# PaddleCV-SIG/MedicalSeg

Hardware: AMD Instinct MI355X
Metric: 3D-voxels/sec fwd+bwd, VNet 128^3 fp32 (higher is better)
Workload: dtype f32

## Files before the change

### include/msegk.h

```cpp
#ifndef MSEGK_H
#define MSEGK_H

#include <stddef.h>
#include <stdint.h>

#ifdef __cplusplus
extern "C" {
#endif

typedef struct msk_ctx msk_ctx;

typedef struct {
  void* p;
  int32_t n, d, h, w, c;
  int32_t ld;
} msk_tensor;

typedef struct {
  int32_t kd, kh, kw;
  int32_t sd, sh, sw;
  int32_t pd, ph, pw;
} msk_conv_desc;

int msk_version(void);
// ... 79 lines not shown
                                 const float* alpha, const float* mean, const float* invstd, msk_tensor dout, float* sums,
                                 float* maxes , int clear_maxes, float* dgamma, float* dbeta, float* dalpha);
int msk_add_act_join_bwd_pg(msk_ctx* ctx, msk_tensor y, const float* scale, const float* shift, const float* alpha_inner,
                            msk_tensor res, const float* alpha_outer, const float* mean, const float* invstd, msk_tensor dout,
                            msk_tensor da, msk_tensor dres, int dres_accumulate, float* dalpha_outer, float* unit_sums,
                            float* maxes , int clear_maxes, float* unit_dgamma, float* unit_dbeta, float* unit_dalpha);
size_t msk_conv3d_bwd_bnact_bytes(msk_ctx* ctx, msk_conv_desc cd, msk_tensor x, msk_tensor y);
int msk_conv3d_bwd_bnact(msk_ctx* ctx, msk_conv_desc cd, msk_tensor x, const float* w, msk_tensor y, const float* scale,
                         const float* shift, const float* alpha , const float* mean, const float* invstd,
                         const float* gamma, msk_tensor dout, const float* sums_total, double M_total,
                         msk_tensor dy_scratch, msk_tensor dx, int dx_accumulate, float* dw, int dw_accumulate,
                         const void* xform , void* ybuf ,
                         const float* maxes );
int msk_conv3d_bwd_bnact_split(msk_ctx* ctx, msk_conv_desc cd, msk_tensor x, const float* w, msk_tensor y, const float* scale,
                               const float* shift, const float* alpha , const float* mean, const float* invstd,
                               const float* gamma, msk_tensor dout, const float* sums_total, double M_total,
                               msk_tensor dy_scratch, msk_tensor dx, int dx_accumulate, float* dw, int dw_accumulate,
                               const void* xform , void* ybuf , const float* maxes ,
                               msk_tensor dx_lo, msk_tensor dx_hi, int* split_done);
int msk_conv3d_bwd_bnact_acc(msk_ctx* ctx, msk_conv_desc cd, msk_tensor x, const float* w, msk_tensor y, const float* scale,
                             const float* shift, const float* alpha, const float* mean, const float* invstd, const float* gamma,
                             msk_tensor dout, const float* sums_total, double M_total, msk_tensor dy_scratch, msk_tensor dx,
                             int dx_accumulate, float* dw, int dw_accumulate, const void* xform, void* ybuf, const float* maxes,
                             msk_tensor dx_old, msk_tensor dx_lo, msk_tensor dx_hi, int* split_done);
int msk_conv3d_bwd_bnact_join(msk_ctx* ctx, msk_conv_desc cd, msk_tensor x, const float* w, msk_tensor y, const float* scale,
                              const float* shift, const float* alpha , const float* mean, const float* invstd,
                              const float* gamma, msk_tensor dout, const float* sums_total, double M_total, msk_tensor dy,
                              float* dy_amax , float* dw, int dw_accumulate, const void* xform ,
                              const float* x_amax , msk_tensor jy, const float* jscale, const float* jshift,
                              const float* jalpha_inner, msk_tensor jres, const float* jalpha_outer, const float* jmean,
                              const float* jinvstd, msk_tensor da, int da_accumulate, msk_tensor dres ,
                              int dres_accumulate, float* dalpha_outer, float* unit_sums, float* maxes, int clear_maxes,
                              float* unit_dgamma , float* unit_dbeta , float* unit_dalpha );
int msk_convT3d_bwd_bnact(msk_ctx* ctx, msk_conv_desc cd, msk_tensor x, const float* w, msk_tensor y, const float* scale,
                          const float* shift, const float* alpha , const float* mean, const float* invstd,
                          msk_tensor dout, const float* sums_total, double M_total, msk_tensor dy_scratch, msk_tensor dx,
                          int dx_accumulate, float* dw, int dw_accumulate);
int msk_conv3d_bwd_inact(msk_ctx* ctx, msk_conv_desc cd, msk_tensor x, const float* w, msk_tensor y, const float* scale,
                         const float* shift, const float* alpha , const float* mean, const float* invstd, int coef_stride,
                         msk_tensor dout, const float* sums, int sums_stride, double M_sample, msk_tensor dx, int dx_accumulate,
                         float* dw, int dw_accumulate, const void* xform, void* ybuf, const float* maxes );
int msk_conv3d_bwd_bnact_c1(msk_ctx* ctx, msk_conv_desc cd, msk_tensor x, msk_tensor y, const float* scale, const float* shift,
                            const float* alpha , const float* mean, const float* invstd, msk_tensor res,
                            msk_tensor dout, const float* sums_total, double M_total, float* dw, int dw_accumulate);
int msk_conv3d_dgrad(msk_ctx* ctx, msk_conv_desc cd, msk_tensor dy, const float* w,
                     msk_tensor dx, int accumulate);
int msk_conv3d_wgrad(msk_ctx* ctx, msk_conv_desc cd, msk_tensor x, msk_tensor dy,
                     float* dw, float* db , int accumulate);
int msk_convT3d_fwd(msk_ctx* ctx, msk_conv_desc cd, msk_tensor x, const float* w,
                    const float* bias , msk_tensor y);
int msk_convT3d_fwd_ex(msk_ctx* ctx, msk_conv_desc cd, msk_tensor x, const float* w, const float* bias, msk_tensor y,
                       float* stats_local, const msk_bn_fin* fin );
int msk_convT3d_dgrad(msk_ctx* ctx, msk_conv_desc cd, msk_tensor dy, const float* w,
                      msk_tensor dx, int accumulate);
int msk_convT3d_wgrad(msk_ctx* ctx, msk_conv_desc cd, msk_tensor x, msk_tensor dy,
                      float* dw, float* db , int accumulate);

int msk_bn_stats(msk_ctx* ctx, msk_tensor x, float* stats_local);
int msk_bn_finalize(msk_ctx* ctx, const float* gathered, int world, double count_per_rank,
                    int C, const float* gamma, const float* beta, float eps, float momentum,
                    float* running_mean, float* running_var, float* save_mean,
                    float* save_invstd, float* scale, float* shift);
int msk_bn_eval_coeffs(msk_ctx* ctx, int C, const float* gamma, const float* beta,
                       const float* running_mean, const float* running_var, float eps,
                       float* save_mean, float* save_invstd, float* scale, float* shift);
int msk_affine_act_fwd(msk_ctx* ctx, msk_tensor x, const float* scale, const float* shift,
// ... 230 lines not shown
```

### medicalseg_amd/_lib.py

```python
from __future__ import annotations

import ctypes as C
import os

_HERE = os.path.dirname(os.path.abspath(__file__))
LIB_PATH = os.environ.get("MSEGK_LIB") or os.path.join(_HERE, "lib", "libmsegk.so")


class MskError(RuntimeError):
    pass


class MskTensor(C.Structure):
    _fields_ = [("p", C.c_void_p), ("n", C.c_int32), ("d", C.c_int32), ("h", C.c_int32),
                ("w", C.c_int32), ("c", C.c_int32), ("ld", C.c_int32)]


class MskConvDesc(C.Structure):
    _fields_ = [("kd", C.c_int32), ("kh", C.c_int32), ("kw", C.c_int32),
                ("sd", C.c_int32), ("sh", C.c_int32), ("sw", C.c_int32),
                ("pd", C.c_int32), ("ph", C.c_int32), ("pw", C.c_int32)]


class MskBnFin(C.Structure):
# ... 36 lines not shown
    "msk_mark_elapsed": (_i, [_vp, _i, _i, C.POINTER(_f)]),
    "msk_prof_enable": (_i, [_vp, _i]),
    "msk_prof_reset": (_i, [_vp]),
    "msk_prof_report": (_i, [_vp, C.c_char_p, _i, C.POINTER(_i)]),
    "msk_set_option": (_i, [_vp, C.c_char_p, _i]),
    "msk_get_option": (_i, [_vp, C.c_char_p, C.POINTER(_i)]),
    "msk_ncdhw_to_ndhwc": (_i, [_vp, _vp, _T]),
    "msk_ndhwc_to_ncdhw": (_i, [_vp, _T, _vp]),
    "msk_conv3d_fwd": (_i, [_vp, _CD, _T, _vp, _vp, _T]),
    "msk_conv_fold_bn": (_i, [_vp, _vp, _vp, _vp, _vp, _i, C.c_long, _vp, _vp]),
    "msk_conv3d_fwd_act": (_i, [_vp, _CD, _T, _vp, _vp, _vp, _T]),
    "msk_conv3d_xform_bytes": (_sz, [_vp, _CD, _T, _i]),
    "msk_conv3d_fwd_ex": (_i, [_vp, _CD, _T, _vp, _vp, _T, _vp, _vp]),
    "msk_conv3d_wgrad_ex": (_i, [_vp, _CD, _T, _T, _vp, _vp, _i, _vp]),
    "msk_amax_new": (_vp, [_vp, _i]),
    "msk_conv3d_fwd_ex3": (_i, [_vp, _CD, _T, _vp, _vp, _T, _vp, _vp, _vp, _vp]),
    "msk_conv3d_fwd_in": (_i, [_vp, _CD, _T, _vp, _vp, _T, _vp, _vp, _vp, _vp, _i]),
    "msk_bn_stats_fin": (_i, [_vp, _T, _vp, _vp]),
    "msk_affine_act_bwd_reduce_pg": (_i, [_vp, _T, _vp, _vp, _T, _vp, _vp, _vp, _T, _vp, _vp, _i, _vp, _vp, _vp]),
    "msk_add_act_join_bwd_pg": (_i, [_vp, _T, _vp, _vp, _vp, _T, _vp, _vp, _vp, _T, _T, _T, _i, _vp, _vp, _vp, _i, _vp, _vp, _vp]),
    "msk_conv3d_fwd_ex2": (_i, [_vp, _CD, _T, _vp, _vp, _T, _vp, _vp, _vp]),
    "msk_affine_act_fwd_amax": (_i, [_vp, _T, _vp, _vp, _T, _vp, _T, _vp]),
    "msk_affine_act_fwd_amax2": (_i, [_vp, _T, _vp, _vp, _T, _vp, _T, _vp, _T]),
    "msk_affine_act_join_fwd_amax": (_i, [_vp, _T, _vp, _vp, _vp, _T, _vp, _T, _vp]),
    "msk_copy_scale_amax": (_i, [_vp, _T, _vp, _T, _i, _vp]),
    "msk_conv3d_bwd_bnact_bytes": (_sz, [_vp, _CD, _T, _T]),
    "msk_conv3d_bwd_bnact": (_i, [_vp, _CD, _T, _vp, _T, _vp, _vp, _vp, _vp, _vp, _vp, _T, _vp, _d, _T, _T, _i, _vp, _i, _vp, _vp, _vp]),
    "msk_convT3d_bwd_bnact": (_i, [_vp, _CD, _T, _vp, _T, _vp, _vp, _vp, _vp, _vp, _T, _vp, _d, _T, _T, _i, _vp, _i]),
    "msk_conv3d_bwd_bnact_split": (_i, [_vp, _CD, _T, _vp, _T, _vp, _vp, _vp, _vp, _vp, _vp, _T, _vp, _d, _T, _T, _i, _vp, _i, _vp, _vp, _vp, _T, _T, C.POINTER(_i)]),
    "msk_conv3d_bwd_bnact_acc": (_i, [_vp, _CD, _T, _vp, _T, _vp, _vp, _vp, _vp, _vp, _vp, _T, _vp, _d, _T, _T, _i, _vp, _i, _vp, _vp, _vp, _T, _T, _T, C.POINTER(_i)]),
    "msk_conv3d_bwd_inact": (_i, [_vp, _CD, _T, _vp, _T, _vp, _vp, _vp, _vp, _vp, _i, _T, _vp, _i, _d, _T, _i, _vp, _i, _vp, _vp, _vp]),
    "msk_conv3d_bwd_bnact_join": (_i, [_vp, _CD, _T, _vp, _T, _vp, _vp, _vp, _vp, _vp, _vp, _T, _vp, _d, _T, _vp, _vp, _i, _vp, _vp,
                                       _T, _vp, _vp, _vp, _T, _vp, _vp, _vp, _T, _i, _T, _i, _vp, _vp, _vp, _i, _vp, _vp, _vp]),
    "msk_conv3d_bwd_bnact_c1": (_i, [_vp, _CD, _T, _T, _vp, _vp, _vp, _vp, _vp, _T, _T, _vp, _d, _vp, _i]),
    "msk_conv3d_dgrad": (_i, [_vp, _CD, _T, _vp, _T, _i]),
    "msk_conv3d_dgrad_ex": (_i, [_vp, _CD, _T, _vp, _T, _i, _vp]),
    "msk_conv3d_wgrad_ex2": (_i, [_vp, _CD, _T, _T, _vp, _vp, _i, _vp, _vp]),
    "msk_conv3d_wgrad_ex3": (_i, [_vp, _CD, _T, _T, _vp, _vp, _i, _vp, _vp, _vp]),
    "msk_conv3d_wgrad": (_i, [_vp, _CD, _T, _T, _vp, _vp, _i]),
    "msk_convT3d_fwd": (_i, [_vp, _CD, _T, _vp, _vp, _T]),
    "msk_convT3d_fwd_ex": (_i, [_vp, _CD, _T, _vp, _vp, _T, _vp, _vp]),
    "msk_convT3d_dgrad": (_i, [_vp, _CD, _T, _vp, _T, _i]),
    "msk_convT3d_wgrad": (_i, [_vp, _CD, _T, _T, _vp, _vp, _i]),
    "msk_bn_stats": (_i, [_vp, _T, _vp]),
    "msk_bn_finalize": (_i, [_vp, _vp, _i, _d, _i, _vp, _vp, _f, _f, _vp, _vp, _vp, _vp, _vp, _vp]),
    "msk_bn_eval_coeffs": (_i, [_vp, _i, _vp, _vp, _vp, _vp, _f, _vp, _vp, _vp, _vp]),
    "msk_affine_act_fwd": (_i, [_vp, _T, _vp, _vp, _T, _vp, _T]),
    "msk_affine_act_bwd_reduce": (_i, [_vp, _T, _vp, _vp, _T, _vp, _vp, _vp, _T, _vp]),
    "msk_affine_act_bwd_reduce_ex": (_i, [_vp, _T, _vp, _vp, _T, _vp, _vp, _vp, _T, _vp, _vp]),
    "msk_affine_act_bwd_apply": (_i, [_vp, _T, _vp, _vp, _T, _vp, _vp, _vp, _vp, _T, _vp, _d, _i, _T, _T, _i]),
    "msk_affine_act_bwd_apply_amax": (_i, [_vp, _T, _vp, _vp, _T, _vp, _vp, _vp, _vp, _T, _vp, _d, _i, _T, _T, _i, _vp]),
    "msk_affine_act_param_grads": (_i, [_vp, _i, _vp, _vp, _vp, _vp, _i]),
    "msk_add_act_bwd": (_i, [_vp, _T, _T, _vp, _T, _T, _T, _i, _vp]),
    "msk_affine_act_join_fwd": (_i, [_vp, _T, _vp, _vp, _vp, _T, _vp, _T]),
    "msk_add_act_join_bwd": (_i, [_vp, _T, _vp, _vp, _vp, _T, _vp, _T, _T, _T, _i, _vp]),
    "msk_add_act_join_bwd_ex": (_i, [_vp, _T, _vp, _vp, _vp, _T, _vp, _vp, _vp, _T, _T, _T, _i, _vp, _vp, _vp]),
    "msk_bn_bias_grad": (_i, [_vp, _i, _vp, _vp, _vp, _i]),
    "msk_copy_scale": (_i, [_vp, _T, _vp, _T, _i]),
    "msk_dropout_mask": (_i, [_vp, _u64, _u64, _u32, _i, _f, _vp]),
    "msk_channel_sum": (_i, [_vp, _T, _vp, _i]),
    "msk_argmax_c": (_i, [_vp, _T, _vp]),
    "msk_softmax_c": (_i, [_vp, _T, _T]),
    "msk_flip_axes": (_i, [_vp, _T, _T, _i]),
    "msk_tta_accumulate": (_i, [_vp, _T, _i, _T, _i]),
    "msk_tta_finish": (_i, [_vp, _T, _i, _T, _vp]),
    "msk_sw_gather": (_i, [_vp, _T, _T, _vp, _f]),
# ... 120 lines not shown
```

### medicalseg_amd/csrc/msk_common.h

```cpp
#pragma once
#include <hip/hip_runtime.h>
#include <hip/hip_ext.h>

#include <cstdint>
#include <cstdio>
#include <cstring>
#include <map>
#include <set>
#include <string>
#include <utility>
#include <vector>

#include "msegk.h"

struct msk_prof_entry {
  double total_ms = 0.0;
  long calls = 0;
};

struct msk_pending_event {
  hipEvent_t a, b;
  const char* tag;
};

// ... 87 lines not shown
  struct { float* param = nullptr; const float* grad = nullptr; float* velocity = nullptr; size_t count = 0;
           float lr = 0, momentum = 0, weight_decay = 0, grad_scale = 0; } late_piece;
  int late_split = 1;
  bool wgrad_async = false;
  bool side_dirty = false;
  hipEvent_t fork_event = nullptr;
  int fork_attach = 1;
  bool fork_recorded = false;
  void* stage[2] = {nullptr, nullptr};
  size_t stage_bytes[2] = {0, 0};
  hipEvent_t stage_ev[2] = {nullptr, nullptr};
  int stage_next = 0;
  void* comm = nullptr;
  void* comm_grad = nullptr;
  hipStream_t comm_stream = nullptr;
  hipEvent_t ev_comm_main = nullptr, ev_comm_side = nullptr, ev_comm_done = nullptr, ev_comm_back = nullptr;
  int c1_h2 = 1;
  int dst_split = 1;
  int wgrad_reduce_rows = 1;
  int ks_stats = 1;
  int ks_lds = 1;
  int ks_nr_max = 4;
  int wgrad_lds_pad = 0;
  int kst_pair = 1;
  int tile_staging = 7;
  int wgrad_renorm = 1;
  int dy_bound_shift = 0;
  int dp_mode = 0;
  bool comm_pending = false;
  bool host_transport = false;
  std::vector<int> host_fds;
  int rank = 0, world = 1;
  int tk_join = 1;
  int topk_agg_hist = 0;
  int affine_map = 1;
  int num_cu = 256;
};

extern thread_local std::string g_msk_global_err;

int msk_fail(msk_ctx* ctx, const char* file, int line, const char* what, const char* detail);
void* msk_workspace(msk_ctx* ctx, size_t bytes);
void* msk_workspace2(msk_ctx* ctx, size_t bytes);
void* msk_workspace3(msk_ctx* ctx, size_t bytes);
hipEvent_t msk_prof_event(msk_ctx* ctx);
void msk_prof_begin(msk_ctx* ctx, const char* tag);
void msk_prof_end(msk_ctx* ctx);
const char* msk_intern_tag(msk_ctx* ctx, const std::string& s);
int msk_join_side_impl(msk_ctx* ctx);
void msk_set_dense12(int v);
void msk_set_reduce_vpl(int v);
void msk_set_reduce_vpl_site(int v);
void msk_set_ew_caps(int ew, int red);
int msk_get_ew_option(const char* key, int* value);
void msk_weights_changed_impl(msk_ctx* ctx, const void* p, size_t bytes);
void msk_weights_freed_impl(msk_ctx* ctx, const void* p, size_t bytes);
int msk_prepack_impl(msk_ctx* ctx);
int msk_prepack_range_impl(msk_ctx* ctx, const void* p, size_t bytes);
int msk_dp_wait_impl(msk_ctx* ctx);
int msk_edt_field(msk_ctx* ctx, const int32_t* vol, int d, int h, int w, int cls, int surface_only, int complement,
                  const double* spacing, double* dist2);
int msk_join_sums_merge(msk_ctx* ctx, const float* partial, int nb, int C, float* unit_sums, float* u_dbeta, float* u_dgamma,
                        float* u_dalpha, float* dalpha);

struct msk_side_scope {
  msk_ctx* ctx;
// ... 91 lines not shown
```

### medicalseg_amd/csrc/msk_ctx.hip

```cpp
#include <cstdlib>

#include "msk_common.h"

thread_local std::string g_msk_global_err;

int msk_fail(msk_ctx* ctx, const char* file, int line, const char* what, const char* detail) {
  char buf[1024];
  const char* base = strrchr(file, '/');
  snprintf(buf, sizeof(buf), "%s:%d: %s: %s", base ? base + 1 : file, line, what, detail ? detail : "");
  if (ctx) ctx->err = buf;
  g_msk_global_err = buf;
  return -1;
}

static void* grow(msk_ctx* ctx, void** p, size_t* cur, size_t bytes) {
  if (bytes <= *cur) return *p;
  if (*p) {
    hipStreamSynchronize(ctx->stream);
    hipFree(*p);
    *p = nullptr;
    *cur = 0;
  }
  size_t want = bytes + (bytes >> 2);
  if (hipMalloc(p, want) != hipSuccess) {
// ... 572 lines not shown
  }
  if (strcmp(key, "ks_legacy") == 0) {
    ctx->ks_legacy = value;
    return 0;
  }
  if (strcmp(key, "wgrad_fork") == 0) {
    ctx->wgrad_fork = value;
    return 0;
  }
  if (strcmp(key, "wbf_fuse") == 0) {
    ctx->wbf_fuse = value;
    return 0;
  }
  if (strcmp(key, "wbf_fused_bl") == 0) {
    ctx->wbf_fused_bl = value;
    return 0;
  }
  if (strcmp(key, "wbf_tpb") == 0) {
    ctx->wbf_tpb = value > 0 ? value : 0;
    return 0;
  }
  if (strcmp(key, "conv_split") == 0) {
    ctx->conv_split = value == 2 ? 2 : 3;
    return 0;
  }
  if (strcmp(key, "bwd_fuse") == 0) {
    ctx->bwd_fuse = value < 0 ? -1 : (value > 2 ? 2 : value);
    return 0;
  }
  if (strcmp(key, "tk_join") == 0) {
    ctx->tk_join = value != 0;
    return 0;
  }
  if (strcmp(key, "affine_map") == 0) {
    ctx->affine_map = value != 0;
    return 0;
  }
  if (strcmp(key, "topk_agg_hist") == 0) {
    ctx->topk_agg_hist = value != 0;
    return 0;
  }
  if (strcmp(key, "foldn_wgs") == 0) {
    ctx->foldn_wgs = value > 0 ? value : 0;
    return 0;
  }
  if (strcmp(key, "wgrad_wino_rounds") == 0) {
    ctx->wgrad_wino_rounds = value > 0 ? value : 0;
    return 0;
  }
  if (strcmp(key, "wgrad_rounds") == 0) {
    ctx->wgrad_rounds = value > 0 ? value : 8;
    return 0;
  }
  if (strcmp(key, "wgrad_chunk") == 0) {
    ctx->wgrad_chunk = value;
    return 0;
  }
  if (strcmp(key, "wgrad_async") == 0) {
    if (msk_join_side_impl(ctx) != 0) return -1;
    ctx->wgrad_async = value != 0;
    return 0;
  }
  if (strcmp(key, "prof_shapes") == 0) {
    ctx->prof_shapes = value != 0;
    return 0;
  }
// ... 14 lines not shown
```

### medicalseg_amd/models/vnet.py

```python
from __future__ import annotations

import os

import numpy as np

from .. import nn
from ..cvlibs import manager
from ..device import Tensor, get_device, to_tensor
from ..nn import AddAct, ConvBNAct, copy_scale

DENSE_TWIN = os.environ.get("MSEGK_DENSE_TWIN", "1") != "0"
SPLIT_CONCAT_GRAD = os.environ.get("MSEGK_SPLIT_CONCAT_GRAD", "1") != "0"


class LUConv(nn.Layer):

    def __init__(self, nchan, elu):
        super(LUConv, self).__init__()
        self.relu1 = nn.ELU() if elu else nn.PReLU(nchan)
        self.conv1 = nn.Conv3D(nchan, nchan, kernel_size=5, padding=2)
        self.bn1 = nn.BatchNorm3D(nchan)
        self._unit = ConvBNAct(self.conv1, self.bn1, self.relu1)

    def forward(self, x):
# ... 176 lines not shown
            op.backward(op._unit.out.grad)
        nn.materialize_grad(xcat)
        gcat = xcat.grad
        split_done = g_lo is not None and getattr(first, "dx_split_done", False)
        if first is not None:
            first.dx_split = None
        if split_done:
            skip.grad = g_hi
        elif self._skip_in_place and skip.grad is None:
            skip.grad = gcat.channel_slice(half, self.outChans)
        else:
            sg = skip.ensure_grad()
            copy_scale(gcat.channel_slice(half, self.outChans), self._m2, sg, accumulate=skip.grad_written)
        skip.grad_written = True
        self._up.backward(g_lo if split_done else gcat.channel_slice(0, half))
        if self._m1 is not None:
            x = self._x
            xg = x.ensure_grad()
            copy_scale(self._xin.grad, self._m1, xg, accumulate=x.grad_written)
            x.grad_written = True


class OutputTransition(nn.Layer):

    def __init__(self, in_channels, num_classes, elu):
        super(OutputTransition, self).__init__()
        self.conv1 = nn.Conv3D(in_channels, num_classes, kernel_size=5, padding=2)
        self.bn1 = nn.BatchNorm3D(num_classes)
        self.conv2 = nn.Conv3D(num_classes, num_classes, kernel_size=1)
        self.relu1 = nn.ELU() if elu else nn.PReLU(num_classes)
        self._unit = ConvBNAct(self.conv1, self.bn1, self.relu1)

    def forward(self, x):
        o = self._unit.forward(x)
        self._o = o
        return self.conv2.run_forward(o)

    def backward(self, dlogits, join=None):
        self.conv2.run_backward(self._o, dlogits, need_dx=True)
        self._unit.backward(self._o.grad, join=join)


@manager.MODELS.add_component
class VNet(nn.Layer):

    def __init__(self, elu=False, in_channels=1, num_classes=4, pretrained=None,
                 kernel_size=((2, 2, 2), (2, 2, 2), (2, 2, 2), (2, 2, 2)),
                 stride_size=((2, 2, 2), (2, 2, 2), (2, 2, 2), (2, 2, 2))):
        super().__init__()
        self.best_loss = 1000000
        self.num_classes = num_classes
        self.in_channels = in_channels

        self.in_tr = InputTransition(in_channels, elu=elu)
        self.down_tr32 = DownTransition(16, 1, elu, downsample_stride=stride_size[0], kernel=kernel_size[0])
        self.down_tr64 = DownTransition(32, 2, elu, downsample_stride=stride_size[1], kernel=kernel_size[1])
        self.down_tr128 = DownTransition(64, 3, elu, dropout=True, downsample_stride=stride_size[2],
                                         kernel=kernel_size[2])
        self.down_tr256 = DownTransition(128, 2, elu, dropout=True, downsample_stride=stride_size[3],
                                         kernel=kernel_size[3])
        self.up_tr256 = UpTransition(256, 256, 2, elu, dropout=True, dropout2=True,
                                     upsample_stride_size=stride_size[3], kernel=kernel_size[3])
        self.up_tr128 = UpTransition(256, 128, 2, elu, dropout=True, dropout2=True,
                                     upsample_stride_size=stride_size[2], kernel=kernel_size[2])
        self.up_tr64 = UpTransition(128, 64, 1, elu, upsample_stride_size=stride_size[1], kernel=kernel_size[1])
        self.up_tr32 = UpTransition(64, 32, 1, elu, upsample_stride_size=stride_size[0], kernel=kernel_size[0])
        self.out_tr = OutputTransition(32, num_classes, elu)

        self.pretrained = pretrained
        self._post_backward_hooks = []
        self._grad_ready_hooks = []
        self._build()
# ... 102 lines not shown
```

### medicalseg_amd/nn.py

```python
from __future__ import annotations

import ctypes as C
import os
import warnings
from collections import OrderedDict

import numpy as np

from . import _lib
from ._lib import NULL_TENSOR, MskBnFin, MskConvDesc, MskError
from .device import Tensor, get_device
from .optimizer import ClipGradByGlobalNorm, ClipGradByNorm, ClipGradByValue

BN_EPS = 1e-5
BN_MOMENTUM = 0.9


def _triple(v):
    if isinstance(v, (list, tuple)):
        if len(v) != 3:
            raise ValueError(f"expected 3 values, got {v}")
        return tuple(int(i) for i in v)
    return (int(v),) * 3

# ... 507 lines not shown
                gathered, nstat = sc["stats"], 1
                if multi:
                    dev.call("msk_dp_allgather", _fp(sc["stats"]), _fp(sc["gathered"]), C.c_size_t(2 * Cn))
                    gathered, nstat = sc["gathered"], dev.world
                dev.call("msk_bn_finalize", _fp(gathered), nstat, C.c_double(y.voxels), Cn, _fp(bn.weight.ptr),
                         _fp(bn.bias.ptr), C.c_float(bn.epsilon), C.c_float(bn.momentum), _fp(bn._mean.ptr),
                         _fp(bn._variance.ptr), _fp(sc["mean"]), _fp(sc["invstd"]), _fp(sc["scale"]), _fp(sc["shift"]))
            self.bn_mode = 1
        else:
            dev.call("msk_bn_eval_coeffs", Cn, _fp(bn.weight.ptr), _fp(bn.bias.ptr), _fp(bn._mean.ptr),
                     _fp(bn._variance.ptr), C.c_float(bn.epsilon), _fp(sc["mean"]), _fp(sc["invstd"]),
                     _fp(sc["scale"]), _fp(sc["shift"]))
            self.bn_mode = 2
        if out is None:
            out = y.empty_like()
        alpha = _act_alpha(self.act)
        if defer_act and res is None and alpha is not None:
            self.deferred = True
        else:
            if isinstance(self.act, ELU):
                dev.call("msk_affine_act_fwd", y.msk(), _fp(sc["scale"]), _fp(sc["shift"]),
                         res.msk() if res is not None else NULL_TENSOR, _fp(alpha), out.msk())
                dev.call("msk_elu_fwd", out.msk(), C.c_float(self.act.alpha), out.msk())
                out.amax = None
            elif out2 is not None:
                dev.call("msk_affine_act_fwd_amax2", y.msk(), _fp(sc["scale"]), _fp(sc["shift"]),
                         res.msk() if res is not None else NULL_TENSOR, _fp(alpha), out.msk(), _amax_for(out), out2.msk())
                out2.amax = out.amax
            else:
                dev.call("msk_affine_act_fwd_amax", y.msk(), _fp(sc["scale"]), _fp(sc["shift"]),
                         res.msk() if res is not None else NULL_TENSOR, _fp(alpha), out.msk(), _amax_for(out))
        self.out = out
        return out

    def backward(self, dout: Tensor, need_dx=True, res_needs_grad=True, join=None):
        if self.bn_mode == 3:
            raise RuntimeError("backward through a forward pass run under nn.fused_inference() (BN folded into the "
                               "convolution: no pre-activation tensor was kept)")
        dev = dout.dev
        bn, sc = self.bn, self.bn.scratch(dev)
        Cn = bn.num_features
        y, res = self.y, self.res
        alpha = _act_alpha(self.act)
        if isinstance(self.act, ELU):
            g = Tensor.empty(dev, dout.n, dout.d, dout.h, dout.w, dout.c)
            dev.call("msk_elu_bwd", self.out.msk(), dout.msk(), C.c_float(self.act.alpha), g.msk(), 0)
            dout = g
        resm = res.msk() if res is not None else NULL_TENSOR
        fuse = (FUSE_BN_BACKWARD and type(self.conv) is Conv3D and res is None and self.bn_mode == 1 and need_dx
                and self.conv.cin == self.conv.cout)
        if not fuse:
            materialize_grad(self.x)
        want_maxes = fuse and Cn % 4 == 0 and y.ld % 4 == 0 and dout.ld % 4 == 0 and y.ptr % 16 == 0 and dout.ptr % 16 == 0
        pg_done = False
        maxes = sc["maxes"]
        if getattr(self, "presummed", False):
            self.presummed = False
            want_maxes = fuse
            pg_done = getattr(self, "presummed_pg", False)
            maxes = getattr(self, "presummed_maxes", None) or sc["maxes"]
        elif want_maxes and FUSE_SMALL:
            maxes = dev.amax_new(2)
            dev.call("msk_affine_act_bwd_reduce_pg", y.msk(), _fp(sc["scale"]), _fp(sc["shift"]), resm, _fp(alpha),
                     _fp(sc["mean"]), _fp(sc["invstd"]), dout.msk(), _fp(sc["sums"]), _fp(maxes), 0,
                     _fp(bn.weight.grad_ptr), _fp(bn.bias.grad_ptr), _fp(_act_alpha_grad(self.act)))
            pg_done = True
# ... 82 lines not shown
            dx = x.ensure_grad()
            rc = dev.lib.msk_convT3d_bwd_bnact(dev.ctx, conv.desc(), x.msk(), _fp(conv.weight.ptr), y.msk(), _fp(sc["scale"]),
                                               _fp(sc["shift"]), _fp(alpha), _fp(sc["mean"]), _fp(sc["invstd"]), dout.msk(),
                                               _fp(sums_total), C.c_double(m_total), dy.msk(), dx.msk(),
                                               1 if x.grad_written else 0, _fp(conv.weight.grad_ptr), 1)
            if rc < 0:
                raise MskError(f"msk_convT3d_bwd_bnact failed: {_lib.last_error(dev.ctx)}")
            if rc == 0:
                _count_flops(conv, x.n, x.d * x.h * x.w, 2)
                x.grad_written = True
                self.dy = dy
                return
        if (join is not None and res is None and need_dx and type(self.conv) is Conv3D and self.bn_mode == 1
                and not isinstance(self.act, ELU) and self.conv.s == (1, 1, 1)
                and join[0].backward_in_dgrad(self, join[1], dout, dy, sums_total, m_total)):
            self.dy = dy
            return
        dres = NULL_TENSOR
        dres_acc = 0
        if res is not None and res_needs_grad and res.c == y.c:
            g = res.ensure_grad()
            dres, dres_acc = g.msk(), 1 if res.grad_written else 0
            res.grad_written = True
        dya = _amax_for(dy) if type(self.conv) is Conv3D and self.conv.s == (1, 1, 1) else None
        dev.call("msk_affine_act_bwd_apply_amax", y.msk(), _fp(sc["scale"]), _fp(sc["shift"]), resm, _fp(alpha),
                 _fp(sc["mean"]), _fp(sc["invstd"]), _fp(bn.weight.ptr), dout.msk(), _fp(sums_total),
                 C.c_double(m_total), self.bn_mode, dy.msk(), dres, dres_acc, dya)
        self.dy = dy
        if self.bn_mode == 2:
            dev.call("msk_bn_bias_grad", Cn, _fp(sc["sums"]), _fp(sc["scale"]), _fp(self.conv.bias.grad_ptr), 1)
        self.conv.run_backward(self.x, dy, need_dx=need_dx, bias_grad=False)


class AddAct:

    def __init__(self, act: PReLU):
        self.act = act
        self._sums = None

    def forward(self, a: Tensor, b: Tensor, unit: "ConvBNAct | None" = None, out: Tensor | None = None) -> Tensor:
        self.a, self.b = a, b
        self._bwd_done = False
        self.unit = unit if (unit is not None and getattr(unit, "deferred", False)) else None
        if out is None:
            out = a.empty_like()
        if isinstance(self.act, ELU):
            a.dev.call("msk_affine_act_fwd", a.msk(), None, None, b.msk(), None, out.msk())
            a.dev.call("msk_elu_fwd", out.msk(), C.c_float(self.act.alpha), out.msk())
            out.amax = None
            self.out = out
            return out
        if self.unit is not None:
            u, sc = self.unit, self.unit.bn.scratch(a.dev)
            a.dev.call("msk_affine_act_join_fwd_amax", u.y.msk(), _fp(sc["scale"]), _fp(sc["shift"]), _fp(u.act._weight.ptr),
                       b.msk(), _fp(self.act._weight.ptr), out.msk(), _amax_for(out))
        else:
            a.dev.call("msk_affine_act_fwd_amax", a.msk(), None, None, b.msk(), _fp(self.act._weight.ptr), out.msk(),
                       _amax_for(out))
        self.out = out
        return out

    def backward_in_dgrad(self, consumer: "ConvBNAct", share_b, dout: Tensor, dy: Tensor, sums_total, m_total) -> bool:
        dev = dout.dev
        a, b, u = self.a, self.b, getattr(self, "unit", None)
        x, conv = consumer.x, consumer.conv
        if getattr(dev.lib.msk_conv3d_bwd_bnact_join, "missing", False):
# ... 103 lines not shown
```

Before: 256.8 million.

## Fuse VNet output head BN-PReLU with 1x1 conv in forward and backward

Adds dedicated head kernels that fuse the final unit's BN affine, PReLU and the small 1x1x1 conv (C<=4) into one pass. The forward skips materializing the activated tensor, and the backward computes dout, the BN/PReLU reduction sums and the conv weight/bias grads in one fused pass with a small merge kernel. This cuts several memory passes and launches over the full-resolution low-channel tensors, which are bandwidth bound. The cost is a deferred-activation path, with fallbacks to the old kernels when shapes or exports don't match.

```diff
diff --git a/include/msegk.h b/include/msegk.h
--- a/include/msegk.h
+++ b/include/msegk.h
@@ -135,6 +135,12 @@
                               const float* jinvstd, msk_tensor da, int da_accumulate, msk_tensor dres ,
                               int dres_accumulate, float* dalpha_outer, float* unit_sums, float* maxes, int clear_maxes,
                               float* unit_dgamma , float* unit_dbeta , float* unit_dalpha );
+int msk_head_fwd(msk_ctx* ctx, msk_tensor y, const float* scale, const float* shift, const float* alpha, const float* w2,
+                 const float* b2 , msk_tensor logits);
+int msk_head_bwd(msk_ctx* ctx, msk_tensor y, msk_tensor dz, const float* scale, const float* shift, const float* mean,
+                 const float* invstd, const float* alpha, const float* w2, msk_tensor dout, float* sums, float* dgamma ,
+                 float* dbeta , float* dalpha , float* dw2, int dw2_accumulate, float* db2 ,
+                 int db2_accumulate);
 int msk_convT3d_bwd_bnact(msk_ctx* ctx, msk_conv_desc cd, msk_tensor x, const float* w, msk_tensor y, const float* scale,
                           const float* shift, const float* alpha , const float* mean, const float* invstd,
                           msk_tensor dout, const float* sums_total, double M_total, msk_tensor dy_scratch, msk_tensor dx,
diff --git a/medicalseg_amd/_lib.py b/medicalseg_amd/_lib.py
--- a/medicalseg_amd/_lib.py
+++ b/medicalseg_amd/_lib.py
@@ -92,6 +92,8 @@
     "msk_conv3d_bwd_inact": (_i, [_vp, _CD, _T, _vp, _T, _vp, _vp, _vp, _vp, _vp, _i, _T, _vp, _i, _d, _T, _i, _vp, _i, _vp, _vp, _vp]),
     "msk_conv3d_bwd_bnact_join": (_i, [_vp, _CD, _T, _vp, _T, _vp, _vp, _vp, _vp, _vp, _vp, _T, _vp, _d, _T, _vp, _vp, _i, _vp, _vp,
                                        _T, _vp, _vp, _vp, _T, _vp, _vp, _vp, _T, _i, _T, _i, _vp, _vp, _vp, _i, _vp, _vp, _vp]),
+    "msk_head_fwd": (_i, [_vp, _T, _vp, _vp, _vp, _vp, _vp, _T]),
+    "msk_head_bwd": (_i, [_vp, _T, _T, _vp, _vp, _vp, _vp, _vp, _vp, _T, _vp, _vp, _vp, _vp, _vp, _i, _vp, _i]),
     "msk_conv3d_bwd_bnact_c1": (_i, [_vp, _CD, _T, _T, _vp, _vp, _vp, _vp, _vp, _T, _T, _vp, _d, _vp, _i]),
     "msk_conv3d_dgrad": (_i, [_vp, _CD, _T, _vp, _T, _i]),
     "msk_conv3d_dgrad_ex": (_i, [_vp, _CD, _T, _vp, _T, _i, _vp]),
diff --git a/medicalseg_amd/csrc/msk_common.h b/medicalseg_amd/csrc/msk_common.h
--- a/medicalseg_amd/csrc/msk_common.h
+++ b/medicalseg_amd/csrc/msk_common.h
@@ -143,6 +143,7 @@
   std::vector<int> host_fds;
   int rank = 0, world = 1;
   int tk_join = 1;
+  int head_fuse = 1;
   int topk_agg_hist = 0;
   int affine_map = 1;
   int num_cu = 256;
diff --git a/medicalseg_amd/csrc/msk_ctx.hip b/medicalseg_amd/csrc/msk_ctx.hip
--- a/medicalseg_amd/csrc/msk_ctx.hip
+++ b/medicalseg_amd/csrc/msk_ctx.hip
@@ -628,6 +628,10 @@
     ctx->tk_join = value != 0;
     return 0;
   }
+  if (strcmp(key, "head_fuse") == 0) {
+    ctx->head_fuse = value < 0 ? 0 : (value > 2 ? 2 : value);
+    return 0;
+  }
   if (strcmp(key, "affine_map") == 0) {
     ctx->affine_map = value != 0;
     return 0;
diff --git a/medicalseg_amd/csrc/msk_head.hip b/medicalseg_amd/csrc/msk_head.hip
--- /dev/null
+++ b/medicalseg_amd/csrc/msk_head.hip
@@ -0,0 +1,329 @@
+#include "msk_common.h"
+#include "msk_conv.h"
+
+namespace {
+
+constexpr int kThreads = 256;
+#ifndef HEAD_BWD_INFLIGHT
+#define HEAD_BWD_INFLIGHT 2
+#endif
+
+template <int C> struct HeadGeom {
+  static constexpr int G = (C == 3) ? 12 : 4;
+  static constexpr int VG = G / C;
+  static constexpr int NACC = 3 * C + C * C + C;
+};
+
+template <int G>
+__device__ __forceinline__ void ldg(const float* __restrict__ p, float (&v)[G]) {
+  const float4* q = reinterpret_cast<const float4*>(p);
+#pragma unroll
+  for (int i = 0; i < G / 4; ++i) {
+    const float4 a = q[i];
+    v[4 * i] = a.x; v[4 * i + 1] = a.y; v[4 * i + 2] = a.z; v[4 * i + 3] = a.w;
+  }
+}
+template <int G>
+__device__ __forceinline__ void stg(float* __restrict__ p, const float (&v)[G]) {
+  float4* q = reinterpret_cast<float4*>(p);
+#pragma unroll
+  for (int i = 0; i < G / 4; ++i) q[i] = make_float4(v[4 * i], v[4 * i + 1], v[4 * i + 2], v[4 * i + 3]);
+}
+
+template <int C>
+struct HeadCoef {
+  float sc[C], sf[C], al[C], w[C * C];
+  template <bool FWD>
+  __device__ __forceinline__ void load(const float* __restrict__ scale, const float* __restrict__ shift,
+                                       const float* __restrict__ alpha, const float* __restrict__ wp) {
+#pragma unroll
+    for (int c = 0; c < C; ++c) { sc[c] = scale[c]; sf[c] = shift[c]; al[c] = alpha[c]; }
+#pragma unroll
+    for (int n = 0; n < C; ++n)
+#pragma unroll
+      for (int c = 0; c < C; ++c) w[n * C + c] = FWD ? wp[c * C + n] : wp[n * C + c];
+  }
+};
+
+template <int C>
+__device__ __forceinline__ void head_fwd_voxel(const HeadCoef<C>& k, const float (&bs)[C], const float* y, float* z) {
+  float o[C];
+#pragma unroll
+  for (int c = 0; c < C; ++c) {
+    const float u = fmaf(y[c], k.sc[c], k.sf[c]);
+    o[c] = !(u > 0.f) ? k.al[c] * u : u;
+  }
+#pragma unroll
+  for (int n = 0; n < C; ++n) {
+    float acc = bs[n];
+#pragma unroll
+    for (int c = 0; c < C; ++c) acc = fmaf(o[c], k.w[n * C + c], acc);
+    z[n] = acc + 0.f;
+  }
+}
+
+template <int C>
+__global__ void __launch_bounds__(kThreads)
+head_fwd_k(const float* __restrict__ y, const float* __restrict__ scale, const float* __restrict__ shift,
+           const float* __restrict__ alpha, const float* __restrict__ wp , const float* __restrict__ b2,
+           float* __restrict__ logits, long groups, long voxels) {
+  constexpr int G = HeadGeom<C>::G, VG = HeadGeom<C>::VG;
+  HeadCoef<C> k;
+  k.template load<true>(scale, shift, alpha, wp);
+  float bs[C];
+#pragma unroll
+  for (int n = 0; n < C; ++n) bs[n] = b2 ? b2[n] : 0.f;
+  for (long g = (long)blockIdx.x * kThreads + threadIdx.x; g < groups; g += (long)gridDim.x * kThreads) {
+    float v[G], z[G];
+    ldg<G>(y + G * g, v);
+#pragma unroll
+    for (int j = 0; j < VG; ++j) head_fwd_voxel<C>(k, bs, v + j * C, z + j * C);
+    stg<G>(logits + G * g, z);
+  }
+  if (blockIdx.x == 0 && threadIdx.x == 0) {
+    for (long m = groups * VG; m < voxels; ++m) {
+      float v[C], z[C];
+#pragma unroll
+      for (int c = 0; c < C; ++c) v[c] = y[m * C + c];
+      head_fwd_voxel<C>(k, bs, v, z);
+#pragma unroll
+      for (int c = 0; c < C; ++c) logits[m * C + c] = z[c];
+    }
+  }
+}
+
+template <int C>
+__global__ void __launch_bounds__(kTpvThreads)
+head_fwd_tpv_k(const float* __restrict__ y, const float* __restrict__ scale, const float* __restrict__ shift,
+               const float* __restrict__ alpha, const float* __restrict__ wp , const float* __restrict__ b2,
+               float* __restrict__ logits, long voxels) {
+  __shared__ float4 tile[tpv_tile_quads(4, 2)];
+  HeadCoef<C> k;
+  k.template load<true>(scale, shift, alpha, wp);
+  float bs[C];
+#pragma unroll
+  for (int n = 0; n < C; ++n) bs[n] = b2 ? b2[n] : 0.f;
+  const long tiles = (voxels + kTpvThreads - 1) / kTpvThreads;
+  for (long t = blockIdx.x; t < tiles; t += gridDim.x) {
+    const long v0 = t * kTpvThreads;
+    const int nv = voxels - v0 < kTpvThreads ? (int)(voxels - v0) : kTpvThreads;
+    tpv_fill<4, 2>(tile, y + v0 * C, nv, C);
+    const bool mine = (int)threadIdx.x < nv;
+    float zz[4], z[4] = {0.f, 0.f, 0.f, 0.f};
+    if (mine) {
+      tpv_take<4, 2>(zz, tile, nullptr, C);
+      head_fwd_voxel<C>(k, bs, zz, z);
+    }
+    tpv_put<4, 2>(z, tile, logits + v0 * C, C, nv, mine, false);
+  }
+}
+
+template <int C>
+__device__ __forceinline__ void head_bwd_voxel(const HeadCoef<C>& k, const float (&mu)[C], const float (&is)[C], const float* y,
+                                               const float* dz, float* dout, float (&acc)[HeadGeom<C>::NACC]) {
+  float u[C], o[C];
+#pragma unroll
+  for (int c = 0; c < C; ++c) {
+    u[c] = fmaf(y[c], k.sc[c], k.sf[c]);
+    o[c] = !(u[c] > 0.f) ? k.al[c] * u[c] : u[c];
+  }
+#pragma unroll
+  for (int c = 0; c < C; ++c) {
+    float d = 0.f;
+#pragma unroll
+    for (int n = 0; n < C; ++n) d = fmaf(dz[n], k.w[n * C + c], d);
+    dout[c] = d;
+    float du = d;
+    if (!(u[c] > 0.f)) {
+      du = k.al[c] * d;
+      acc[2 * C + c] = fmaf(d, u[c], acc[2 * C + c]);
+    }
+    acc[c] += du;
+    acc[C + c] = fmaf(du, (y[c] - mu[c]) * is[c], acc[C + c]);
+  }
+#pragma unroll
+  for (int n = 0; n < C; ++n) {
+#pragma unroll
+    for (int c = 0; c < C; ++c) acc[3 * C + n * C + c] = fmaf(dz[n], o[c], acc[3 * C + n * C + c]);
+    acc[3 * C + C * C + n] += dz[n];
+  }
+}
+
+template <int C>
+__global__ void __launch_bounds__(kThreads)
+head_bwd_k(const float* __restrict__ y, const float* __restrict__ dz, const float* __restrict__ scale,
+           const float* __restrict__ shift, const float* __restrict__ mean, const float* __restrict__ invstd,
+           const float* __restrict__ alpha, const float* __restrict__ wp , float* __restrict__ dout, long groups,
+           long voxels, float* __restrict__ partial ) {
+  constexpr int G = HeadGeom<C>::G, VG = HeadGeom<C>::VG, NACC = HeadGeom<C>::NACC;
+  HeadCoef<C> k;
+  k.template load<false>(scale, shift, alpha, wp);
+  float mu[C], is[C];
+#pragma unroll
+  for (int c = 0; c < C; ++c) { mu[c] = mean[c]; is[c] = invstd[c]; }
+  float acc[NACC];
+#pragma unroll
+  for (int i = 0; i < NACC; ++i) acc[i] = 0.f;
+  const long per = (groups + gridDim.x - 1) / gridDim.x;
+  const long g0 = (long)blockIdx.x * per;
+  long g1 = g0 + per;
+  if (g1 > groups) g1 = groups;
+  long g = g0 + threadIdx.x;
+#if HEAD_BWD_INFLIGHT == 2
+  for (; g + kThreads < g1; g += 2 * kThreads) {
+    float va[G], da[G], vb[G], db[G], oa[G], ob[G];
+    ldg<G>(y + G * g, va);
+    ldg<G>(dz + G * g, da);
+    ldg<G>(y + G * (g + kThreads), vb);
+    ldg<G>(dz + G * (g + kThreads), db);
+#pragma unroll
+    for (int j = 0; j < VG; ++j) head_bwd_voxel<C>(k, mu, is, va + j * C, da + j * C, oa + j * C, acc);
+    stg<G>(dout + G * g, oa);
+#pragma unroll
+    for (int j = 0; j < VG; ++j) head_bwd_voxel<C>(k, mu, is, vb + j * C, db + j * C, ob + j * C, acc);
+    stg<G>(dout + G * (g + kThreads), ob);
+  }
+#endif
+  for (; g < g1; g += kThreads) {
+    float v[G], d[G], o[G];
+    ldg<G>(y + G * g, v);
+    ldg<G>(dz + G * g, d);
+#pragma unroll
+    for (int j = 0; j < VG; ++j) head_bwd_voxel<C>(k, mu, is, v + j * C, d + j * C, o + j * C, acc);
+    stg<G>(dout + G * g, o);
+  }
+  if (blockIdx.x == 0 && threadIdx.x == 0) {
+    for (long m = groups * VG; m < voxels; ++m) {
+      float v[C], d[C], o[C];
+#pragma unroll
+      for (int c = 0; c < C; ++c) { v[c] = y[m * C + c]; d[c] = dz[m * C + c]; }
+      head_bwd_voxel<C>(k, mu, is, v, d, o, acc);
+#pragma unroll
+      for (int c = 0; c < C; ++c) dout[m * C + c] = o[c];
+    }
+  }
+  __shared__ float sh[kThreads / 64][NACC];
+  const int lane = threadIdx.x & 63, wave = threadIdx.x >> 6;
+#pragma unroll
+  for (int i = 0; i < NACC; ++i) {
+    float v = acc[i];
+#pragma unroll
+    for (int o = 32; o > 0; o >>= 1) v += __shfl_xor(v, o, 64);
+    if (lane == 0) sh[wave][i] = v;
+  }
+  __syncthreads();
+  if (threadIdx.x < NACC) {
+    float v = 0.f;
+#pragma unroll
+    for (int w = 0; w < kThreads / 64; ++w) v += sh[w][threadIdx.x];
+    partial[(long)blockIdx.x * NACC + threadIdx.x] = v;
+  }
+}
+
+__global__ void __launch_bounds__(256)
+head_sums_merge_k(const float* __restrict__ partial, int nb, int C, int nacc, float* __restrict__ sums, float* __restrict__ dbeta,
+                  float* __restrict__ dgamma, float* __restrict__ dalpha, float* __restrict__ dw2, int dw2_accumulate,
+                  float* __restrict__ db2, int db2_accumulate) {
+  __shared__ double sh[256];
+  const int i = blockIdx.x, t = threadIdx.x, nt = blockDim.x;
+  double s = 0;
+  for (int b = t; b < nb; b += nt) s += partial[(long)b * nacc + i];
+  sh[t] = s;
+  __syncthreads();
+  for (int k = nt >> 1; k > 0; k >>= 1) {
+    if (t < k) sh[t] += sh[t + k];
+    __syncthreads();
+  }
+  if (t != 0) return;
+  const float v = (float)sh[0];
+  if (i < 3 * C) {
+    const int q = i / C, c = i % C;
+    sums[i] = v;
+    float* g = q == 0 ? dbeta : (q == 1 ? dgamma : dalpha);
+    if (g) g[c] += v;
+  } else if (i < 3 * C + C * C) {
+    float* o = dw2 + (i - 3 * C);
+    *o = dw2_accumulate ? *o + v : v;
+  } else if (db2) {
+    float* o = db2 + (i - 3 * C - C * C);
+    *o = db2_accumulate ? *o + v : v;
+  }
+}
+
+inline bool head_dense(const msk_tensor& t, int C) { return t.p != nullptr && t.c == C && t.ld == C && (((uintptr_t)t.p) & 15) == 0; }
+
+}
+
+extern "C" {
+
+int msk_head_fwd(msk_ctx* ctx, msk_tensor y, const float* scale, const float* shift, const float* alpha, const float* w2,
+                 const float* b2, msk_tensor logits) {
+  MSK_REQUIRE(ctx, msk_same_shape(y, logits), "msk_head_fwd: y/logits shape mismatch");
+  const int C = y.c;
+  const long voxels = msk_voxels(y);
+  if (!ctx->head_fuse || C < 1 || C > 4 || voxels < 1 || !alpha || !scale || !shift || !w2 || !head_dense(y, C) || !head_dense(logits, C))
+    return 1;
+  const float* wp = msk_pack_weights_get(ctx, w2, C, C, 1, 1, 0, 1, 1, 1, 0, C, C, 0, 0);
+  if (!wp) return -1;
+  int cap = 4;
+  msk_get_ew_option("ew_cap", &cap);
+  msk_launch_scope ls(ctx, "pointwise_small_bnact");
+  if (ctx->head_fuse == 2) {
+    const dim3 grid(msk_ew_blocks(voxels, ctx->num_cu, cap));
+#define HEAD_TPV(C_) hipLaunchKernelGGL(head_fwd_tpv_k<C_>, grid, dim3(kTpvThreads), 0, ctx->stream, (const float*)y.p, scale, shift, alpha, \
+                                        wp, b2, (float*)logits.p, voxels)
+    if (C == 1) HEAD_TPV(1); else if (C == 2) HEAD_TPV(2); else if (C == 3) HEAD_TPV(3); else HEAD_TPV(4);
+#undef HEAD_TPV
+    MSK_LAUNCH_CHECK(ctx);
+    return 0;
+  }
+#define HEAD_FWD(C_)                                                                                                         \
+  do {                                                                                                                        \
+    const long groups = voxels / HeadGeom<C_>::VG;                                                                            \
+    hipLaunchKernelGGL(head_fwd_k<C_>, dim3(msk_ew_blocks(groups, ctx->num_cu, cap)), dim3(kThreads), 0, ctx->stream,         \
+                       (const float*)y.p, scale, shift, alpha, wp, b2, (float*)logits.p, groups, voxels);                     \
+  } while (0)
+  if (C == 1) HEAD_FWD(1); else if (C == 2) HEAD_FWD(2); else if (C == 3) HEAD_FWD(3); else HEAD_FWD(4);
+#undef HEAD_FWD
+  MSK_LAUNCH_CHECK(ctx);
+  return 0;
+}
+
+int msk_head_bwd(msk_ctx* ctx, msk_tensor y, msk_tensor dz, const float* scale, const float* shift, const float* mean,
+                 const float* invstd, const float* alpha, const float* w2, msk_tensor dout, float* sums, float* dgamma,
+                 float* dbeta, float* dalpha, float* dw2, int dw2_accumulate, float* db2, int db2_accumulate) {
+  MSK_REQUIRE(ctx, msk_same_shape(y, dz) && msk_same_shape(y, dout), "msk_head_bwd: y/dz/dout shape mismatch");
+  const int C = y.c;
+  const long voxels = msk_voxels(y);
+  if (!ctx->head_fuse || C < 1 || C > 4 || voxels < 1 || !alpha || !scale || !shift || !mean || !invstd || !w2 || !sums || !dw2 ||
+      !head_dense(y, C) || !head_dense(dz, C) || !head_dense(dout, C))
+    return 1;
+  const float* wp = msk_pack_weights_get(ctx, w2, C, C, 1, 0, 0, 1, 1, 1, 0, C, C, 0, 0);
+  if (!wp) return -1;
+  int cap = 4;
+  msk_get_ew_option("reduce_cap", &cap);
+  const int nacc = 3 * C + C * C + C;
+  const long groups = voxels / (C == 3 ? 4 : 4 / C);
+  if (cap > 2) cap = 2;
+  long nb = (groups + 2 * kThreads - 1) / (2 * kThreads);
+  if (nb > (long)ctx->num_cu * cap) nb = (long)ctx->num_cu * cap;
+  if (nb < 1) nb = 1;
+  float* partial = (float*)msk_workspace(ctx, (size_t)nb * nacc * sizeof(float));
+  if (!partial) return -1;
+  {
+    msk_launch_scope ls(ctx, "wgrad_pw_small_bnact");
+#define HEAD_BWD(C_)                                                                                                          \
+  hipLaunchKernelGGL(head_bwd_k<C_>, dim3((unsigned)nb), dim3(kThreads), 0, ctx->stream, (const float*)y.p, (const float*)dz.p, \
+                     scale, shift, mean, invstd, alpha, wp, (float*)dout.p, groups, voxels, partial)
+    if (C == 1) HEAD_BWD(1); else if (C == 2) HEAD_BWD(2); else if (C == 3) HEAD_BWD(3); else HEAD_BWD(4);
+#undef HEAD_BWD
+    MSK_LAUNCH_CHECK(ctx);
+  }
+  msk_launch_scope ls(ctx, "sums_merge");
+  hipLaunchKernelGGL(head_sums_merge_k, dim3(nacc), dim3(nb > 256 ? 256 : 64), 0, ctx->stream, partial, (int)nb, C, nacc, sums,
+                     dbeta, dgamma, dalpha, dw2, dw2_accumulate, db2, db2_accumulate);
+  MSK_LAUNCH_CHECK(ctx);
+  return 0;
+}
+
+}
diff --git a/medicalseg_amd/models/vnet.py b/medicalseg_amd/models/vnet.py
--- a/medicalseg_amd/models/vnet.py
+++ b/medicalseg_amd/models/vnet.py
@@ -232,12 +232,15 @@
         self._unit = ConvBNAct(self.conv1, self.bn1, self.relu1)
 
     def forward(self, x):
-        o = self._unit.forward(x)
-        self._o = o
-        return self.conv2.run_forward(o)
+        self._o, logits, self._head_fused = nn.head_forward(self._unit, self.conv2, x)
+        return logits
 
     def backward(self, dlogits, join=None):
-        self.conv2.run_backward(self._o, dlogits, need_dx=True)
+        if not (self._head_fused and nn.head_backward(self._unit, self.conv2, self._o, dlogits)):
+            if self._head_fused:
+                self._unit.apply_deferred_act()
+            self.conv2.run_backward(self._o, dlogits, need_dx=True)
+        self._head_fused = False
         self._unit.backward(self._o.grad, join=join)
 
 
diff --git a/medicalseg_amd/nn.py b/medicalseg_amd/nn.py
--- a/medicalseg_amd/nn.py
+++ b/medicalseg_amd/nn.py
@@ -563,6 +563,14 @@
                          res.msk() if res is not None else NULL_TENSOR, _fp(alpha), out.msk(), _amax_for(out))
         self.out = out
         return out
+
+    def apply_deferred_act(self):
+        if not self.deferred:
+            return
+        sc, out = self.bn.scratch(self.y.dev), self.out
+        out.dev.call("msk_affine_act_fwd_amax", self.y.msk(), _fp(sc["scale"]), _fp(sc["shift"]), NULL_TENSOR,
+                     _fp(_act_alpha(self.act)), out.msk(), _amax_for(out))
+        self.deferred = False
 
     def backward(self, dout: Tensor, need_dx=True, res_needs_grad=True, join=None):
         if self.bn_mode == 3:
@@ -711,6 +719,66 @@
         self.conv.run_backward(self.x, dy, need_dx=need_dx, bias_grad=False)
 
 
+_HEAD_WARNED = {"done": False}
+
+
+def _head_entry_points(dev):
+    lib = dev.lib
+    if getattr(lib.msk_head_fwd, "missing", False) or getattr(lib.msk_head_bwd, "missing", False):
+        if not _HEAD_WARNED["done"]:
+            _HEAD_WARNED["done"] = True
+            warnings.warn(f"{_lib.LIB_PATH} does not export msk_head_fwd / msk_head_bwd: the tail of the output block runs as "
+                          "separate kernels; rebuild with ./build.sh", RuntimeWarning)
+        return None
+    return lib.msk_head_fwd, lib.msk_head_bwd
+
+
+def head_forward(unit: ConvBNAct, conv2: Conv3D, x: Tensor):
+    dev = x.dev
+    small = isinstance(unit.act, PReLU) and conv2.cin == conv2.cout == unit.conv.cout <= 4 and conv2.k == (1, 1, 1) \
+        and conv2.s == (1, 1, 1) and conv2.p == (0, 0, 0)
+    entry = _head_entry_points(dev) if small else None
+    if entry is None:
+        o = unit.forward(x)
+        return o, conv2.run_forward(o), False
+    o = unit.forward(x, defer_act=True)
+    if not unit.deferred:
+        return o, conv2.run_forward(o), False
+    y, sc = unit.y, unit.bn.scratch(dev)
+    logits = y.empty_like()
+    rc = entry[0](dev.ctx, y.msk(), _fp(sc["scale"]), _fp(sc["shift"]), _fp(_act_alpha(unit.act)), _fp(conv2.weight.ptr),
+                  _fp(conv2.bias.ptr), logits.msk())
+    if rc < 0:
+        raise MskError(f"msk_head_fwd failed: {_lib.last_error(dev.ctx)}")
+    if rc != 0:
+        unit.apply_deferred_act()
+        return o, conv2.run_forward(o, logits), False
+    _count_flops(conv2, y.n, y.d * y.h * y.w, 1)
+    return o, logits, True
+
+
+def head_backward(unit: ConvBNAct, conv2: Conv3D, o: Tensor, dlogits: Tensor) -> bool:
+    dev = dlogits.dev
+    entry = _head_entry_points(dev)
+    if entry is None or not unit.deferred or o.grad_written:
+        return False
+    bn, sc, y = unit.bn, unit.bn.scratch(dev), unit.y
+    do = o.ensure_grad()
+    rc = entry[1](dev.ctx, y.msk(), dlogits.msk(), _fp(sc["scale"]), _fp(sc["shift"]), _fp(sc["mean"]), _fp(sc["invstd"]),
+                  _fp(_act_alpha(unit.act)), _fp(conv2.weight.ptr), do.msk(), _fp(sc["sums"]), _fp(bn.weight.grad_ptr),
+                  _fp(bn.bias.grad_ptr), _fp(_act_alpha_grad(unit.act)), _fp(conv2.weight.grad_ptr), 1,
+                  _fp(conv2.bias.grad_ptr), 1)
+    if rc < 0:
+        raise MskError(f"msk_head_bwd failed: {_lib.last_error(dev.ctx)}")
+    if rc != 0:
+        return False
+    _count_flops(conv2, y.n, y.d * y.h * y.w, 2)
+    o.grad_written = True
+    do.amax = None
+    unit.presummed, unit.presummed_pg, unit.presummed_maxes = True, True, None
+    return True
+
+
 class AddAct:
 
     def __init__(self, act: PReLU):
```

Result: no change. 257.5 million, median of 6 (+0.3%).
